# fnzhan/EMLight

Measured on AMD Instinct MI355X. Metric: training images/sec (regression step: DenseNet-BC fwd + Sinkhorn loss + bwd + Adam), higher is better.
Workload: dtype f32; 1 GPU; RegressionNetwork train step, BASELINE configs[1]; per_gpu_batch=64, global_batch=64, anchors=128, parallelism=single

## Files before the change

emlight_amd/RegressionNetwork/dense_engine_bwd.py:

```python
import ctypes
import os

import torch

from .. import _lib
from .._knobs import knob_choice, knob_flag


def _r16(v):
    return (v + 15) // 16 * 16


def _side_stream(dev, prio):
    if prio <= 0:
        return torch.cuda.Stream(device=dev, priority=prio)
    hip = ctypes.CDLL("libamdhip64.so")
    h = ctypes.c_void_p()
    with torch.cuda.device(dev):
        rc = hip.hipStreamCreateWithPriority(ctypes.byref(h), ctypes.c_uint(1), ctypes.c_int(prio))
    if rc != 0:
        raise RuntimeError("hipStreamCreateWithPriority failed (%d)" % rc)
    return torch.cuda.ExternalStream(h.value, device=dev)


def _masked_stream(dev, n_cu, keep):
    hip = ctypes.CDLL("libamdhip64.so")
    words = (n_cu + 31) // 32
    mask = (ctypes.c_uint32 * words)()
    for i in range(n_cu):
        if keep(i):
            mask[i // 32] |= 1 << (i % 32)
    h = ctypes.c_void_p()
    with torch.cuda.device(dev):
        rc = hip.hipExtStreamCreateWithCUMask(ctypes.byref(h), ctypes.c_uint32(words), mask)
    if rc != 0:
        raise RuntimeError("hipExtStreamCreateWithCUMask failed (%d)" % rc)
    return torch.cuda.ExternalStream(h.value, device=dev)


class _BwdBuffers:
    def __init__(self, enc, ws, dev):
        f32 = dict(dtype=torch.float32, device=dev)
        self.G = [torch.zeros(blk["P"], blk["ld"], **f32) for blk in ws.blocks]
        self.GF = torch.zeros(ws.F.shape[0], ws.F.shape[1], **f32)
        maxP = ws.blocks[0]["P"]
        self.DZ = torch.empty(2, maxP, 48, **f32)
        self.ring = max(1, int(os.environ.get("EML_WGRAD_RING", 4))) if enc.overlap_wgrad(dev) else 1
        self.GF12 = [torch.empty(maxP, 12, **f32) for _ in range(self.ring)]
        self.N12 = torch.empty(maxP, 12, **f32)
        self.TOP = torch.empty(2 * maxP * 12, **f32) if knob_flag("EML_DGRAD_TOP", True) else None
        kp, ko, g = enc.kp_max, max(enc.ko_max, 48), enc.grid_max
        self.Wd = [[torch.empty(lay["Kp"] * 48, **f32) for lay in blk["layers"]] for blk in ws.blocks]
        self.WdT = [torch.empty(blk["trans"]["Kp"] * blk["trans"]["Ko"], **f32) for blk in ws.blocks]
        self.permutes = None
        self.coef = torch.zeros(8, max(kp, ko), **f32)
        self.part2 = torch.zeros(2, g * kp * 2, dtype=torch.float64, device=dev)
        self.partW = torch.empty(g * max(kp * 48, 2 * 27 * 256, 4 * 1024), **f32)
        i32 = dict(dtype=torch.int32, device=dev)
        self.cond = [[torch.zeros(lay["Kp"], **i32) for lay in blk["layers"]] for blk in ws.blocks]
        self.condT = [torch.zeros(blk["trans"]["Kp"], **i32) for blk in ws.blocks]
        self.any_ill = torch.zeros(1, **i32)
        self.dg_grid = 128
        self.dg_scratch = torch.empty(self.dg_grid * kp, dtype=torch.float64, device=dev)
        self.side = None
        if enc.overlap_wgrad(dev):
            m = int(os.environ.get("EML_CU_SPLIT", 0))
            self.main_masked = None
            if m > 1:
                n_cu = torch.cuda.get_device_properties(dev).multi_processor_count
                self.side = _masked_stream(dev, n_cu, lambda i: i % m == m - 1)
                self.main_masked = _masked_stream(dev, n_cu, lambda i: i % m != m - 1)
# ... 49 lines not shown
        mod_ = getattr(f, "denseblock%d" % (bi_ + 1))
        for l_, lay_ in enumerate(blk_["layers"]):
            items.append((getattr(mod_, "denselayer%d" % (l_ + 1)).conv1.weight, bw.Wd[bi_][l_], 2, 48, lay_["Cin"],
                          lay_["Kp"], 48))
        tr_ = blk_["trans"]
        items.append((getattr(f, "transition%d" % (bi_ + 1)).conv.weight, bw.WdT[bi_], 2, tr_["Cout"], blk_["Ctot"],
                      tr_["Kp"], tr_["Ko"]))
    bw.permutes.launch(L, st, items)
    params = enc.param_list()
    if need_params is None:
        need_params = [True] * len(params)
    from .._dist import grad_slot
    grads = {}
    for q, need in zip(params, need_params):
        slot = grad_slot(q) if need else None
        grads[id(q)] = slot if slot is not None else torch.empty_like(q)
    gr = lambda q: p(grads[id(q)])
    coefs = [tuple(bw.coef[3 * k + i] for i in range(3)) for k in range(2)]
    cA, cB, cC = coefs[0]
    sB, sC = bw.coef[6], bw.coef[7]

    direct = knob_choice("EML_DGAMMA_DIRECT", "always", ("always", "never")) != "never"
    c3_fold = knob_flag("EML_C3_FOLD", True)
    bw.any_ill.zero_()

    def dgamma_direct(blk, X_ld, Pin, Hin, Win, pool, DY, ld_dy, Zr, ld_z, co, Cout, conv, Cin, scale1, shift1, cond, bn):
        if not direct:
            return
        a, b, c = co if co is not None else (None, None, None)
        _lib.check(L.eml_dense_bn_dgamma_direct_f32(
            p(blk["X"]), X_ld, Pin, Hin, Win, pool, p(DY), ld_dy, p(Zr), ld_z, p(a), p(b), p(c), Cout, p(conv.weight), Cin,
            p(scale1), p(shift1), p(blk["mean"]), p(blk["istd"]), p(cond), p(bw.dg_scratch), gr(bn.weight), bw.dg_grid, st),
            "eml_dense_bn_dgamma_direct_f32")

    def finalize(R, pstride, count, bn, mean, istd, C, Cpad, coef=0, s_acc=None, src=None, c_lo=0, c_hi=None, conv=None,
                 cond=None):
        a, b, c = coefs[coef] if coef is not None else (None, None, None)
        wargs = (p(bn.bias), p(conv.weight), gr(conv.weight), conv.weight.shape[0]) if conv is not None else (None, None, None, 0)
        _lib.check(L.eml_dense_bn_bwd_finalize_f32(
            p(part if src is None else src), R, pstride, float(count), p(bn.weight), p(mean), p(istd), C, Cpad, 1,
            gr(bn.weight), gr(bn.bias), p(a), p(b), p(c),
            p(sB) if s_acc is not None else None, p(sC) if s_acc is not None else None, int(bool(s_acc)),
            c_lo, Cpad if c_hi is None else c_hi, *wargs, p(cond), p(bw.any_ill) if cond is not None else None, st),
            "eml_dense_bn_bwd_finalize_f32")

    def parr(tensors):
# ... 29 lines not shown
        _lib.check(L.eml_dense_conv1x1_bwd_data_f32(
            p(dY), ld_dy, p(tr["T"]), Ko, p(cA), p(cB), p(cC), Ko, p(bw.WdT[bi]), None, ld, p(tr["scale"]),
            p(tr["shift"]), None, None, Pn, Hb, Wb, 1, kpt, p(Gbuf), ld, 0, p(part), G, p(tr["mask16"]), st),
            "eml_dense_conv1x1_bwd_data_f32")
        finalize(G, 2 * kpt, P, T.norm, blk["mean"], blk["istd"], ctot, kpt, coef=None, s_acc=False, conv=T.conv,
                 cond=bw.condT[bi])
        dgamma_direct(blk, ld, P, Hb, Wb, 1, dY, ld_dy, tr["T"], Ko, coefs[0], cout, T.conv, ctot, tr["scale"], tr["shift"],
                      bw.condT[bi], T.norm)
        def conv2_backward(l, slot, n12=False, narrow_lo=None, top=False):
            lay = blk["layers"][l]
            Lm = getattr(mod, "denselayer%d" % (l + 1))
            cin, kp, z, dz = lay["Cin"], lay["Kp"], blk["Z"][l], bw.DZ[slot]
            gsrc = (p(bw.N12), 12, 0) if n12 else (p(top2[1]), 12, 0) if top else (p(Gbuf), ld, cin)
            r = ring[0] = (ring[0] + 1) % bw.ring
            if bw.side is not None and bw.ev_done[r] is not None:
                main.wait_event(bw.ev_done[r])
            fold = (bw.side is None and c3_fold
                    and L.eml_dense_conv3x3_bwd_fused_supported(gsrc[1], gsrc[2], ld, cin) == 1)
            q = ws.drop_plan[bi][l] if ws.drop_plan is not None else 0.0
            drop = (ws.drop_key, gl0 + l, q) if q > 0 else ()
            if fold:
                fn = "eml_dense_conv3x3_bwd_fused_drop_f32" if drop else "eml_dense_conv3x3_bwd_fused_f32"
                _lib.check(getattr(L, fn)(*gsrc, p(Lm.conv2.weight), p(z), p(lay["zmean"]), p(lay["zistd"]), p(dz), B, Hb, Wb,
                                          p(part), G3d, p(blk["X"]), ld, cin, p(sB), p(sC), p(bw.GF12[r]), p(lay["scale2"]),
                                          p(lay["shift2"]), p(bw.partW), gr(Lm.conv2.weight), *drop, st), fn)
            else:
                fn = "eml_dense_conv3x3_bwd_data_drop_f32" if drop else "eml_dense_conv3x3_bwd_data_f32"
                _lib.check(getattr(L, fn)(*gsrc, p(Lm.conv2.weight), p(z), p(lay["zmean"]), p(lay["zistd"]), p(dz), B, Hb, Wb,
                                          p(part), G3d, p(blk["X"]), ld, cin, p(sB), p(sC), p(bw.GF12[r]), *drop, st), fn)
            if fold:
                pass
            elif bw.side is None:
                _lib.check(L.eml_dense_conv3x3_bwd_weight_f32(p(bw.GF12[r]), 12, 0, p(z), p(lay["scale2"]),
                                                              p(lay["shift2"]), B, Hb, Wb, p(bw.partW),
                                                              gr(Lm.conv2.weight), G3, st),
                           "eml_dense_conv3x3_bwd_weight_f32")
            else:
                bw.ev_ready[r].record(main)
                bw.side.wait_event(bw.ev_ready[r])
                _lib.check(L.eml_dense_conv3x3_bwd_weight_f32(p(bw.GF12[r]), 12, 0, p(z), p(lay["scale2"]),
                                                              p(lay["shift2"]), B, Hb, Wb, p(bw.partW3[r]),
                                                              gr(Lm.conv2.weight), G3s, st_side),
                           "eml_dense_conv3x3_bwd_weight_f32")
                if bw.ev_done[r] is None:
                    bw.ev_done[r] = torch.cuda.Event()
                bw.ev_done[r].record(bw.side)
            finalize(G3d, 96, P, Lm.norm2, lay["zmean"], lay["zistd"], 48, 48, coef=slot)
            a, b, c = coefs[slot]
            _lib.check(L.eml_dense_conv1x1_bwd_weight_f32(
                p(blk["X"]), ld, P, Hb, Wb, 0, kp, cin, p(lay["scale1"]), p(lay["shift1"]), p(dz), 48, p(z), 48,
                p(a), p(b), p(c), 48, p(bw.partW), gr(Lm.conv1.weight), Gw, p(dz),
                *((p(Lm.conv1.weight), narrow_lo, *((p(top2[0]), 12) if top else (p(Gbuf), ld)), p(bw.N12),
                   p(bw.part2[slot])) if narrow_lo is not None
                  else (None, 0, None, 0, None, None)), st), "eml_dense_conv1x1_bwd_weight_f32")
            return Lm

        def dgrad(layers, slots, k_lo, k_hi, top=False):
            lays = [blk["layers"][l] for l in layers]
            if top:
                _lib.check(L.eml_dense_conv1x1_bwd_data_multi_top_f32(
                    parr([bw.DZ[s_] for s_ in slots]), parr([bw.Wd[bi][l_] for l_ in layers]),
                    parr([y["scale1"] for y in lays]), parr([y["shift1"] for y in lays]),
                    parr([bw.part2[s_] for s_ in slots]), (ctypes.c_int * len(layers))(*[y["Kp"] for y in lays]),
# ... 80 lines not shown
```

emlight_amd/csrc/dense_bwd.hip:

```cpp
#include "eml_common.h"
#include "eml_dropout.h"

#include <cstdint>
#include <cstdlib>
#include <type_traits>

namespace {

using f32x4 = __attribute__((ext_vector_type(4))) float;

__device__ __forceinline__ f32x4 mfma16(float a, float b, f32x4 c) {
  return __builtin_amdgcn_mfma_f32_16x16x4f32(a, b, c, 0, 0, 0);
}
__device__ __forceinline__ float f4c(const float4& v, int t) { return t == 0 ? v.x : t == 1 ? v.y : t == 2 ? v.z : v.w; }
__device__ __forceinline__ double shfl_xor_d(double v, int m) { return __shfl_xor(v, m, 64); }

constexpr int kTH = 8, kTW = 32, kHH = kTH + 2, kHW = kTW + 2;

constexpr int kPSG = 14;
constexpr int kBD = 512;
constexpr int kGRows = 2;
constexpr int kGPass = kHH / kGRows;

template <bool FUSE, bool WIDE, int TH, bool DROP = false>
// ... 420 lines not shown
#pragma unroll
  for (int i = 0; i < 7; ++i) {
    const int idx = w4 + 4 * i;
    if (idx < 27) {
#pragma unroll
      for (int g = 0; g < 4; ++g)
        partial[((((size_t)blockIdx.x * 2 + half) * 27 + idx) * 16 + 4 * kk + g) * 16 + r] = acc[i][g];
    }
  }
}


#ifdef EML_STAMPS
__device__ unsigned long long eml_c3_stamps[8];
#define EML_C3_STAMP(slot)                                                   \
  do {                                                                       \
    const unsigned long long now_ = __builtin_readcyclecounter();            \
    st_acc[slot] += now_ - st_last;                                          \
    st_last = now_;                                                          \
  } while (0)
#else
#define EML_C3_STAMP(slot) do {} while (0)
#endif
template <bool A16, bool DROP = false>
__global__ __launch_bounds__(512, 2) void conv3x3_bwd_fused_kernel(
    const float* __restrict__ G, int ldg, int c0, const float* __restrict__ W2, const float* __restrict__ Z,
    const float* __restrict__ zmean, const float* __restrict__ zistd, float* __restrict__ DZ, int B, int H, int W,
    double* __restrict__ partials , const float* __restrict__ Xb, int ldx, int cx,
    const float* __restrict__ sB, const float* __restrict__ sC, float* __restrict__ GF,
    const float* __restrict__ scale2, const float* __restrict__ shift2, float* __restrict__ partialW ,
    eml::DropKey dk) {
  extern __shared__ __attribute__((aligned(16))) float smem[];
  constexpr int kGT = kHH * kHW * kPSG;
  float* g_l = smem;
  float* z_l = g_l + 2 * kGT;
  float* w_l = z_l + kHH * kHW * kPSW;
  float* coef_l = w_l + 27 * 3 * 64;
  double* red = reinterpret_cast<double*>(coef_l + 32);
  const int tid = threadIdx.x, lane = tid & 63, wave = tid >> 6;
  const int r = lane & 15, kk = lane >> 4;
  const int half = wave >> 2, w4 = wave & 3;

  for (int e = tid; e < 27 * 3 * 64; e += 512) {
    const int l = e & 63, g3 = e >> 6, n = g3 % 3, ts = g3 / 3, s3 = ts % 3, tap = ts / 3;
    w_l[e] = W2[((size_t)(4 * s3 + (l >> 4)) * 48 + 16 * n + (l & 15)) * 9 + tap];
  }
  if (tid < 24) coef_l[tid] = tid < 12 ? sB[cx + tid] : sC[cx + tid - 12];
// ... 17 lines not shown
  for (int it = 0; it < 2; ++it) {
    const int t = min(tid + 512 * it, kWideItems - 1), hp = t / 3;
    w_q[it] = t - 3 * hp;
    w_hy[it] = hp / kHW;
    w_hx[it] = hp - w_hy[it] * kHW;
  }
  float4 gt4[2], xt4[2];
  const int s_hx = min(tid / 12, kHW - 1), s_q = tid % 12;
  const float4 sc = *reinterpret_cast<const float4*>(scale2 + 4 * s_q);
  const float4 sh = *reinterpret_cast<const float4*>(shift2 + 4 * s_q);
  const int s_dst = s_hx * kPSW + 4 * s_q;
  float4 zt[kHH];
  const float* s_src = Z;
  int s_y0 = 0;
  bool s_col = false;
  auto stage_begin = [&](int tile) {
    const int b = tile / (ty_n * tx_n), rem = tile - b * (ty_n * tx_n);
    const int ty = rem / tx_n, tx = rem - ty * tx_n;
#pragma unroll
    for (int it = 0; it < 2; ++it) {
      const int gy = ty * kTH - 1 + w_hy[it], gx = tx * kTW - 1 + w_hx[it];
      w_ok[it] = gy >= 0 && gy < H && gx >= 0 && gx < W;
      w_pix[it] = (b * H + min(max(gy, 0), H - 1)) * W + min(max(gx, 0), W - 1);
      w_own[it] = w_ok[it] && w_hy[it] >= 1 && w_hy[it] <= kTH && w_hx[it] >= 1 && w_hx[it] <= kTW;
    }
    const int gx = tx * kTW - 1 + s_hx;
    s_y0 = ty * kTH - 1;
    s_col = gx >= 0 && gx < W;
    s_src = Z + ((size_t)b * H * W + min(max(gx, 0), W - 1)) * 48 + 4 * s_q;
  };
  auto g_load = [&](int it) {
    const float* gp = G + (size_t)w_pix[it] * ldg + c0 + 4 * w_q[it];
    const float* xp = Xb + (size_t)w_pix[it] * ldx + cx + 4 * w_q[it];
    if constexpr (A16) {
      gt4[it] = *reinterpret_cast<const float4*>(gp);
      xt4[it] = *reinterpret_cast<const float4*>(xp);
    } else {
      const float2 g0 = *reinterpret_cast<const float2*>(gp), g1 = *reinterpret_cast<const float2*>(gp + 2);
      const float2 x0 = *reinterpret_cast<const float2*>(xp), x1 = *reinterpret_cast<const float2*>(xp + 2);
      gt4[it] = make_float4(g0.x, g0.y, g1.x, g1.y);
      xt4[it] = make_float4(x0.x, x0.y, x1.x, x1.y);
    }
  };
  auto g_commit = [&](int it, float* dst) {
    const float4 fb4 = *reinterpret_cast<const float4*>(coef_l + 4 * w_q[it]);
    const float4 fc4 = *reinterpret_cast<const float4*>(coef_l + 12 + 4 * w_q[it]);
    float4 v;
    v.x = fmaf(fb4.x, xt4[it].x, gt4[it].x) + fc4.x;
    v.y = fmaf(fb4.y, xt4[it].y, gt4[it].y) + fc4.y;
    v.z = fmaf(fb4.z, xt4[it].z, gt4[it].z) + fc4.z;
    v.w = fmaf(fb4.w, xt4[it].w, gt4[it].w) + fc4.w;
    if constexpr (DROP) v = eml::drop4(dk, (unsigned)w_pix[it], (unsigned)w_q[it], v);
    if (!w_ok[it]) v = make_float4(0.f, 0.f, 0.f, 0.f);
    float* d = dst + (w_hy[it] * kHW + w_hx[it]) * kPSG + 4 * w_q[it];
    *reinterpret_cast<float2*>(d) = make_float2(v.x, v.y);
    *reinterpret_cast<float2*>(d + 2) = make_float2(v.z, v.w);
    if (w_own[it]) *reinterpret_cast<float4*>(GF + (size_t)w_pix[it] * 12 + 4 * w_q[it]) = v;
  };
  auto z_load = [&](int it) {
    zt[it] = *reinterpret_cast<const float4*>(s_src + (size_t)min(max(s_y0 + it, 0), H - 1) * W * 48);
  };
  auto z_commit = [&](int it, int y0, bool col) {
    const bool ok = col && y0 + it >= 0 && y0 + it < H;
    float4 v;
    v.x = ok ? fmaf(zt[it].x, sc.x, sh.x) : 0.f;
    v.y = ok ? fmaf(zt[it].y, sc.y, sh.y) : 0.f;
    v.z = ok ? fmaf(zt[it].z, sc.z, sh.z) : 0.f;
    v.w = ok ? fmaf(zt[it].w, sc.w, sh.w) : 0.f;
    *reinterpret_cast<float4*>(z_l + s_dst + it * kHW * kPSW) = v;
  };

  int tile = blockIdx.x, cur = 0;
  __syncthreads();
  if (tile < ntiles) {
    stage_begin(tile);
    g_load(0);
    g_load(1);
#pragma unroll
    for (int it = 0; it < kHH; ++it) z_load(it);
    g_commit(0, g_l);
// ... 131 lines not shown
#pragma unroll
  for (int i = 0; i < 7; ++i) {
    const int idx = w4 + 4 * i;
    if (idx < 27) {
#pragma unroll
      for (int g = 0; g < 4; ++g)
        partialW[((((size_t)blockIdx.x * 2 + half) * 27 + idx) * 16 + 4 * kk + g) * 16 + r] = accw[i][g];
    }
  }
  __syncthreads();
  if (tid < 48) {
    double t1 = 0.0, t2 = 0.0;
#pragma unroll
    for (int w8 = 0; w8 < 8; ++w8) {
      t1 += red[(w8 * 48 + tid) * 2 + 0];
      t2 += red[(w8 * 48 + tid) * 2 + 1];
    }
    partials[(size_t)blockIdx.x * 96 + 2 * tid + 0] = t1;
    partials[(size_t)blockIdx.x * 96 + 2 * tid + 1] = (double)zistd[tid] * (t2 - (double)zmean[tid] * t1);
  }
}


template <bool A16, bool DROP = false>
__global__ __launch_bounds__(512, 2) void conv3x3_bwd_fused_tp_kernel(
    const float* __restrict__ G, int ldg, int c0, const float* __restrict__ W2, const float* __restrict__ Z,
    const float* __restrict__ zmean, const float* __restrict__ zistd, float* __restrict__ DZ, int B, int H, int W,
    double* __restrict__ partials , const float* __restrict__ Xb, int ldx, int cx,
    const float* __restrict__ sB, const float* __restrict__ sC, float* __restrict__ GF,
    const float* __restrict__ scale2, const float* __restrict__ shift2, float* __restrict__ partialW ,
    eml::DropKey dk) {
  extern __shared__ __attribute__((aligned(16))) float smem[];
  constexpr int kGT = kHH * kHW * kPSG;
  constexpr int kZS = 48;
  float* g_l = smem;
  float* z_l = g_l + 2 * kGT;
  float* w_l = z_l + 2 * kTH * kTW * kZS;
  float* coef_l = w_l + 27 * 3 * 64;
  double* red = reinterpret_cast<double*>(coef_l + 32);
  const int tid = threadIdx.x, lane = tid & 63, wave = tid >> 6;
  const int r = lane & 15, kk = lane >> 4;

  for (int e = tid; e < 27 * 3 * 64; e += 512) {
    const int l = e & 63, g3 = e >> 6, n = g3 % 3, ts = g3 / 3, s3 = ts % 3, tap = ts / 3;
    w_l[e] = W2[((size_t)(4 * s3 + (l >> 4)) * 48 + 16 * n + (l & 15)) * 9 + tap];
  }
  if (tid < 24) coef_l[tid] = tid < 12 ? sB[cx + tid] : sC[cx + tid - 12];
// ... 25 lines not shown
#pragma unroll
  for (int it = 0; it < 2; ++it) {
    const int t = min(tid + 512 * it, kWideItems - 1), hp = t / 3;
    w_q[it] = t - 3 * hp;
    w_hy[it] = hp / kHW;
    w_hx[it] = hp - w_hy[it] * kHW;
  }
  f32x4 gt4[2], xt4[2];
  constexpr int kZI = kTH * kTW * 12 / 512;
  int z_pq[kZI];
#pragma unroll
  for (int it = 0; it < kZI; ++it) {
    const int t = tid + 512 * it;
    z_pq[it] = ((t / 12) << 4) | (t % 12);
  }
  auto stage_begin = [&](int tile) {
    const int b = tile / (ty_n * tx_n), rem = tile - b * (ty_n * tx_n);
    const int ty = rem / tx_n, tx = rem - ty * tx_n;
#pragma unroll
    for (int it = 0; it < 2; ++it) {
      const int gy = ty * kTH - 1 + w_hy[it], gx = tx * kTW - 1 + w_hx[it];
      w_ok[it] = gy >= 0 && gy < H && gx >= 0 && gx < W;
      w_pix[it] = (b * H + min(max(gy, 0), H - 1)) * W + min(max(gx, 0), W - 1);
      w_own[it] = w_ok[it] && w_hy[it] >= 1 && w_hy[it] <= kTH && w_hx[it] >= 1 && w_hx[it] <= kTW;
    }
  };
  auto g_load = [&](int it) {
    const float* gp = G + (size_t)w_pix[it] * ldg + c0 + 4 * w_q[it];
    const float* xp = Xb + (size_t)w_pix[it] * ldx + cx + 4 * w_q[it];
    if constexpr (A16) {
      asm volatile("global_load_dwordx4 %0, %1, off" : "=&v"(gt4[it]) : "v"(gp) : "memory");
      asm volatile("global_load_dwordx4 %0, %1, off" : "=&v"(xt4[it]) : "v"(xp) : "memory");
    } else {
      const float2 g0 = *reinterpret_cast<const float2*>(gp), g1 = *reinterpret_cast<const float2*>(gp + 2);
      const float2 x0 = *reinterpret_cast<const float2*>(xp), x1 = *reinterpret_cast<const float2*>(xp + 2);
      gt4[it] = f32x4{g0.x, g0.y, g1.x, g1.y};
      xt4[it] = f32x4{x0.x, x0.y, x1.x, x1.y};
    }
  };
  auto g_wait = [&]() {
    if constexpr (A16)
      asm volatile("s_waitcnt vmcnt(0)" : "+v"(gt4[0]), "+v"(xt4[0]), "+v"(gt4[1]), "+v"(xt4[1]) :: "memory");
  };
  auto g_commit = [&](int it, float* dst) {
    const float4 fb4 = *reinterpret_cast<const float4*>(coef_l + 4 * w_q[it]);
    const float4 fc4 = *reinterpret_cast<const float4*>(coef_l + 12 + 4 * w_q[it]);
    float4 v;
    v.x = fmaf(fb4.x, xt4[it][0], gt4[it][0]) + fc4.x;
    v.y = fmaf(fb4.y, xt4[it][1], gt4[it][1]) + fc4.y;
    v.z = fmaf(fb4.z, xt4[it][2], gt4[it][2]) + fc4.z;
    v.w = fmaf(fb4.w, xt4[it][3], gt4[it][3]) + fc4.w;
    if constexpr (DROP) v = eml::drop4(dk, (unsigned)w_pix[it], (unsigned)w_q[it], v);
    if (!w_ok[it]) v = make_float4(0.f, 0.f, 0.f, 0.f);
    float* d = dst + (w_hy[it] * kHW + w_hx[it]) * kPSG + 4 * w_q[it];
    *reinterpret_cast<float2*>(d) = make_float2(v.x, v.y);
    *reinterpret_cast<float2*>(d + 2) = make_float2(v.z, v.w);
    gt4[it] = f32x4{v.x, v.y, v.z, v.w};
  };
  auto g_store = [&](int it) {
    if (w_own[it]) *reinterpret_cast<float4*>(GF + ((unsigned)w_pix[it] * 12u + 4u * (unsigned)w_q[it])) = make_float4(gt4[it][0], gt4[it][1], gt4[it][2], gt4[it][3]);
  };
  auto z_dma = [&](int it, int b, int y0, int x0, int buf) {
    const int pix = z_pq[it] >> 4, q = z_pq[it] & 15;
    const int gy = min(y0 + (pix >> 5), H - 1), gx = min(x0 + (pix & 31), W - 1);
    const float* src = Z + ((size_t)(b * H + gy) * W + gx) * 48 + 4 * q;
    unsigned keep;
    const unsigned dst = __builtin_amdgcn_readfirstlane(
        (unsigned)(size_t)(const __attribute__((address_space(3))) char*)(z_l + buf * (kTH * kTW * kZS) + 4 * (64 * wave + 512 * it)));
    asm volatile("s_mov_b32 %0, m0\n\ts_mov_b32 m0, %2\n\ts_nop 0\n\tglobal_load_lds_dwordx4 %1, off\n\ts_mov_b32 m0, %0"
                 : "=&s"(keep) : "v"(src), "s"(dst) : "memory");
  };

  int tile = blockIdx.x, cur = 0;
  __syncthreads();
  if (tile < ntiles) {
    stage_begin(tile);
    g_load(0);
    g_load(1);
    {
      const int b = tile / (ty_n * tx_n), rem = tile - b * (ty_n * tx_n);
#pragma unroll
      for (int it = 0; it < kZI; ++it) z_dma(it, b, (rem / tx_n) * kTH, (rem % tx_n) * kTW, 0);
// ... 1901 lines not shown
                     (size_t)27 * 256, 1, 0, 0, 0, dW2);
  return eml::check_launch("eml_dense_conv3x3_bwd_weight_f32(reduce)");
}

#ifdef EML_STAMPS
extern "C" int eml_c3_read_stamps(unsigned long long* out, int reset) {
  if (hipMemcpyFromSymbol(out, HIP_SYMBOL(eml_c3_stamps), 8 * sizeof(unsigned long long)) != hipSuccess) return -1;
  if (reset) {
    const unsigned long long z[8] = {0};
    if (hipMemcpyToSymbol(HIP_SYMBOL(eml_c3_stamps), z, sizeof(z)) != hipSuccess) return -1;
  }
  return 0;
}
#endif
extern "C" int eml_dense_conv3x3_bwd_fused_supported(int ldg, int c0, int ldx, int cx) {
  return ((ldg & 1) == 0 && (c0 & 1) == 0 && (ldx & 1) == 0 && (cx & 1) == 0) ? 1 : 0;
}
template <bool DROP>
static int conv3x3_bwd_fused_launch(const char* name, const float* G, int ldg, int c0, const float* W2, const float* Z,
                                    const float* zmean, const float* zistd, float* DZ, int B, int H, int W, double* partials,
                                    int grid, const float* X, int ldx, int cx, const float* sB, const float* sC, float* GF,
                                    const float* scale2, const float* shift2, float* partialW, float* dW2, eml::DropKey dk,
                                    eml_stream_t stream) {
  if (!G || !W2 || !Z || !zmean || !zistd || !DZ || !partials || !X || !sB || !sC || !GF || !scale2 || !shift2 || !partialW ||
      !dW2 || B < 1 || H < 1 || W < 1 || grid < 1 || cx < 0)
    return eml::fail(EML_EINVAL, "%s: bad arguments", name);
  const auto al16 = [](const void* q) { return (reinterpret_cast<uintptr_t>(q) & 15) == 0; };
  if (!eml_dense_conv3x3_bwd_fused_supported(ldg, c0, ldx, cx) || !al16(G) || !al16(X) || !al16(GF) || !al16(Z) || !al16(scale2) ||
      !al16(shift2))
    return eml::fail(EML_EINVAL, "%s: needs even ldg, c0, ldx, cx and 16-byte aligned buffers", name);
  const bool a16 = (ldg & 3) == 0 && (c0 & 3) == 0 && (ldx & 3) == 0 && (cx & 3) == 0;
#ifndef EML_C3_WTP
#define EML_C3_WTP 1
#endif
#if EML_C3_WTP
  const size_t lds = (size_t)(2 * kHH * kHW * kPSG + 2 * kTH * kTW * 48 + 27 * 3 * 64 + 32) * sizeof(float) + 8 * 48 * 2 * sizeof(double);
  if (a16) {
    EML_ENSURE_LDS((&conv3x3_bwd_fused_tp_kernel<true, DROP>), lds);
    hipLaunchKernelGGL((conv3x3_bwd_fused_tp_kernel<true, DROP>), dim3(grid), dim3(512), lds, (hipStream_t)stream, G, ldg, c0, W2, Z,
                       zmean, zistd, DZ, B, H, W, partials, X, ldx, cx, sB, sC, GF, scale2, shift2, partialW, dk);
  } else {
    EML_ENSURE_LDS((&conv3x3_bwd_fused_tp_kernel<false, DROP>), lds);
    hipLaunchKernelGGL((conv3x3_bwd_fused_tp_kernel<false, DROP>), dim3(grid), dim3(512), lds, (hipStream_t)stream, G, ldg, c0, W2, Z,
                       zmean, zistd, DZ, B, H, W, partials, X, ldx, cx, sB, sC, GF, scale2, shift2, partialW, dk);
  }
  int rc = eml::check_launch(name);
  if (rc) return rc;
  hipLaunchKernelGGL(reduce_rows_kernel, dim3(21 * 256 / 64), dim3(256), 0, (hipStream_t)stream, partialW, grid,
                     (size_t)21 * 256, 3, 0, 0, 0, dW2);
  return eml::check_launch(DROP ? "eml_dense_conv3x3_bwd_fused_drop_f32(reduce)" : "eml_dense_conv3x3_bwd_fused_f32(reduce)");
#else
  const size_t lds = (size_t)(2 * kHH * kHW * kPSG + kHH * kHW * kPSW + 27 * 3 * 64 + 32) * sizeof(float) + 8 * 48 * 2 * sizeof(double);
  if (a16) {
    EML_ENSURE_LDS((&conv3x3_bwd_fused_kernel<true, DROP>), lds);
    hipLaunchKernelGGL((conv3x3_bwd_fused_kernel<true, DROP>), dim3(grid), dim3(512), lds, (hipStream_t)stream, G, ldg, c0, W2, Z, zmean,
                       zistd, DZ, B, H, W, partials, X, ldx, cx, sB, sC, GF, scale2, shift2, partialW, dk);
  } else {
    EML_ENSURE_LDS((&conv3x3_bwd_fused_kernel<false, DROP>), lds);
    hipLaunchKernelGGL((conv3x3_bwd_fused_kernel<false, DROP>), dim3(grid), dim3(512), lds, (hipStream_t)stream, G, ldg, c0, W2, Z, zmean,
                       zistd, DZ, B, H, W, partials, X, ldx, cx, sB, sC, GF, scale2, shift2, partialW, dk);
  }
  int rc = eml::check_launch(name);
  if (rc) return rc;
  hipLaunchKernelGGL(reduce_rows_kernel, dim3(27 * 256 / 64), dim3(256), 0, (hipStream_t)stream, partialW, 2 * grid,
                     (size_t)27 * 256, 1, 0, 0, 0, dW2);
  return eml::check_launch(DROP ? "eml_dense_conv3x3_bwd_fused_drop_f32(reduce)" : "eml_dense_conv3x3_bwd_fused_f32(reduce)");
#endif
}

extern "C" int eml_dense_conv3x3_bwd_fused_f32(const float* G, int ldg, int c0, const float* W2, const float* Z,
                                               const float* zmean, const float* zistd, float* DZ, int B, int H, int W,
                                               double* partials, int grid, const float* X, int ldx, int cx,
                                               const float* sB, const float* sC, float* GF, const float* scale2,
                                               const float* shift2, float* partialW, float* dW2, eml_stream_t stream) {
  return conv3x3_bwd_fused_launch<false>("eml_dense_conv3x3_bwd_fused_f32", G, ldg, c0, W2, Z, zmean, zistd, DZ, B, H, W, partials,
                                         grid, X, ldx, cx, sB, sC, GF, scale2, shift2, partialW, dW2, eml::DropKey{}, stream);
}

extern "C" int eml_dense_conv3x3_bwd_fused_drop_f32(const float* G, int ldg, int c0, const float* W2, const float* Z,
                                                    const float* zmean, const float* zistd, float* DZ, int B, int H, int W,
                                                    double* partials, int grid, const float* X, int ldx, int cx,
                                                    const float* sB, const float* sC, float* GF, const float* scale2,
                                                    const float* shift2, float* partialW, float* dW2, unsigned long long seed,
// ... 397 lines not shown
```

emlight_amd/csrc/dense_fwd.hip:

```cpp
#include "eml_common.h"
#include "eml_dropout.h"

namespace {

using f32x4 = __attribute__((ext_vector_type(4))) float;

__device__ __forceinline__ f32x4 mfma16(float a, float b, f32x4 c) {
  return __builtin_amdgcn_mfma_f32_16x16x4f32(a, b, c, 0, 0, 0);
}
__device__ __forceinline__ float f4c(const float4& v, int t) { return t == 0 ? v.x : t == 1 ? v.y : t == 2 ? v.z : v.w; }

__device__ __forceinline__ float4 bn_relu4(float4 x, float4 s, float4 t) {
  float4 r;
  r.x = fmaxf(fmaf(x.x, s.x, t.x), 0.f);
  r.y = fmaxf(fmaf(x.y, s.y, t.y), 0.f);
  r.z = fmaxf(fmaf(x.z, s.z, t.z), 0.f);
  r.w = fmaxf(fmaf(x.w, s.w, t.w), 0.f);
  return r;
}

__device__ __forceinline__ double shfl_xor_d(double v, int m) { return __shfl_xor(v, m, 64); }

template <int NT>
__device__ __forceinline__ void block_stats_store(double (&s)[NT], double (&q)[NT], double* red ,
// ... 219 lines not shown
        __builtin_amdgcn_fence(__ATOMIC_ACQUIRE, "wavefront");
      }
    }
  }
#ifndef EML_FWD_STATS_LDS
#pragma unroll
  for (int n = 0; n < 3; ++n)
#pragma unroll
    for (int g = 0; g < 4; ++g) {
#pragma unroll
      for (int o = 1; o < 16; o <<= 1) {
        ssum[n][g] += shfl_xor_d(ssum[n][g], o);
        ssq[n][g] += shfl_xor_d(ssq[n][g], o);
      }
      if (r == 0) {
        red[(wave * 48 + 16 * n + 4 * kk + g) * 2 + 0] = ssum[n][g];
        red[(wave * 48 + 16 * n + 4 * kk + g) * 2 + 1] = ssq[n][g];
      }
    }
#endif
  __syncthreads();
  for (int e = tid; e < 96; e += 256)
    partials[(size_t)blockIdx.x * 96 + e] = (red[e] + red[96 + e]) + (red[192 + e] + red[288 + e]);
}

constexpr int kTH = 8, kTW = 32;
constexpr int kHH = kTH + 2, kHW = kTW + 2;
constexpr int kPS = 56;

constexpr int kC3Threads = 512;

template <bool DROP>
__global__ __launch_bounds__(kC3Threads) void conv3x3_fwd_kernel(
    const float* __restrict__ Z, const float* __restrict__ scale2, const float* __restrict__ shift2,
    const float* __restrict__ W2p, float* __restrict__ X, int ldx, int c_out0, int B, int H, int W,
    double* __restrict__ partials, eml::DropKey dk) {
  extern __shared__ __attribute__((aligned(16))) float smem[];
  float* st_l = smem + 2 * kHH * kHW * kPS;
  double* red = reinterpret_cast<double*>(st_l + 96);
  const int tid = threadIdx.x, lane = tid & 63, wave = tid >> 6;
  const int r = lane & 15, kk = lane >> 4;

  if (tid < 48) {
    st_l[tid] = scale2[tid];
    st_l[48 + tid] = shift2[tid];
  }
// ... 665 lines not shown
  hipLaunchKernelGGL(permute_w2_kernel, dim3(27), dim3(256), 0, (hipStream_t)stream, W2, Cout, W2p);
  return eml::check_launch("eml_dense_permute_w2_f32");
}

extern "C" int eml_dense_conv1x1_fwd_f32(const float* X, int ldx, long P, int Hin, int Win, int pool, int Kp,
                                         const float* scale, const float* shift, const float* Wp, int Cout,
                                         float* out, int ldo, double* partials, int grid,
                                         unsigned long long* relu_mask, eml_stream_t stream) {
  if (!X || !scale || !shift || !Wp || !out || !partials || P < 1 || grid < 1 || Kp < 16 || (Kp & 15) || Kp > ldx ||
      (ldx & 3) || Cout < 1)
    return eml::fail(EML_EINVAL, "eml_dense_conv1x1_fwd_f32: bad arguments");
  if (relu_mask && (pool || Cout > 48))
    return eml::fail(EML_EINVAL, "eml_dense_conv1x1_fwd_f32: relu_mask is for dense layers (no pool, Cout <= 48)");
  if (pool && ((Hin & 1) || (Win & 1))) return eml::fail(EML_EINVAL, "eml_dense_conv1x1_fwd_f32: pool needs even H, W");
  static const bool staged_env = [] { const char* v = getenv("EML_FWD_STAGED"); return !(v && v[0] == '0'); }();
  const size_t lds0 = ((size_t)Kp * 48 + 2 * Kp) * sizeof(float) + 4 * 48 * 2 * sizeof(double) +
                      (relu_mask ? (size_t)4 * 16 * (Kp / 16) * sizeof(unsigned long long) : 0);
  const size_t stg_bytes = (size_t)4 * 16 * 52 * sizeof(float);
  const int staged = (staged_env && !pool && Cout == 48 && ldo == 48 && (reinterpret_cast<size_t>(out) & 15) == 0 &&
                      lds0 + stg_bytes <= 80 * 1024) ? 1 : 0;
  const size_t lds = lds0 + (staged ? stg_bytes : 0);
  if (lds > 160 * 1024) return eml::fail(EML_EINVAL, "eml_dense_conv1x1_fwd_f32: Kp=%d does not fit LDS", Kp);
  const int nchunks = (Cout + 47) / 48;
  for (int ch = 0; ch < nchunks; ++ch) {
    const int nv = (Cout - ch * 48 < 48) ? Cout - ch * 48 : 48;
    const float* wp = Wp + (size_t)ch * Kp * 48;
    double* pp = partials + (size_t)ch * grid * 96;
    if (pool) {
      EML_ENSURE_LDS((&conv1x1_fwd_kernel<true, false>), lds);
      hipLaunchKernelGGL((conv1x1_fwd_kernel<true, false>), dim3(grid), dim3(256), lds, (hipStream_t)stream, X, ldx, (int)P, Hin,
                         Win, Kp, scale, shift, wp, out + ch * 48, ldo, nv, pp, nullptr, 0);
    } else if (relu_mask) {
      EML_ENSURE_LDS((&conv1x1_fwd_kernel<false, true>), lds);
      hipLaunchKernelGGL((conv1x1_fwd_kernel<false, true>), dim3(grid), dim3(256), lds, (hipStream_t)stream, X, ldx, (int)P,
                         Hin, Win, Kp, scale, shift, wp, out + ch * 48, ldo, nv, pp, relu_mask, staged);
    } else {
      EML_ENSURE_LDS((&conv1x1_fwd_kernel<false, false>), lds);
      hipLaunchKernelGGL((conv1x1_fwd_kernel<false, false>), dim3(grid), dim3(256), lds, (hipStream_t)stream, X, ldx, (int)P,
                         Hin, Win, Kp, scale, shift, wp, out + ch * 48, ldo, nv, pp, nullptr, staged);
    }
    int rc = eml::check_launch("eml_dense_conv1x1_fwd_f32");
    if (rc) return rc;
  }
  return EML_OK;
}

extern "C" int eml_dense_conv3x3_fwd_f32(const float* Z, const float* scale2, const float* shift2, const float* W2p,
// ... 49 lines not shown
```

Baseline: 555.5 images/s.

## Fuse multi-chunk transition 1x1 conv forward into one pass; skip unused GF12 stores

Adds a wide conv1x1 forward kernel that handles two or three 48-channel output chunks per launch, so a transition conv reads and BN-ReLUs its input once instead of once per chunk. Only the 1x1 convs with more than 48 outputs and no pool or relu mask are affected. The fused conv3x3 backward kernels gain a template flag that skips writing the GF12 gradient buffer when the weight-gradient pass is folded in, and by default that buffer is no longer allocated or passed. The wide kernel holds up to 3x the weight tile in LDS at occupancy 1 and carries larger accumulator arrays, which raises register pressure.

Measured after the change: 561.3 images/s (median of 6 runs). +1.0%, better.

```diff
diff --git a/emlight_amd/RegressionNetwork/dense_engine_bwd.py b/emlight_amd/RegressionNetwork/dense_engine_bwd.py
--- a/emlight_amd/RegressionNetwork/dense_engine_bwd.py
+++ b/emlight_amd/RegressionNetwork/dense_engine_bwd.py
@@ -39,6 +39,11 @@
 
 
 class _BwdBuffers:
+    def gf12(self, r):
+        if self.GF12[r] is None:
+            self.GF12[r] = self._gf12_new()
+        return self.GF12[r]
+
     def __init__(self, enc, ws, dev):
         f32 = dict(dtype=torch.float32, device=dev)
         self.G = [torch.zeros(blk["P"], blk["ld"], **f32) for blk in ws.blocks]
@@ -46,7 +51,8 @@
         maxP = ws.blocks[0]["P"]
         self.DZ = torch.empty(2, maxP, 48, **f32)
         self.ring = max(1, int(os.environ.get("EML_WGRAD_RING", 4))) if enc.overlap_wgrad(dev) else 1
-        self.GF12 = [torch.empty(maxP, 12, **f32) for _ in range(self.ring)]
+        self.GF12 = [None] * self.ring
+        self._gf12_new = lambda: torch.empty(maxP, 12, **f32)
         self.N12 = torch.empty(maxP, 12, **f32)
         self.TOP = torch.empty(2 * maxP * 12, **f32) if knob_flag("EML_DGRAD_TOP", True) else None
         kp, ko, g = enc.kp_max, max(enc.ko_max, 48), enc.grid_max
@@ -142,6 +148,7 @@
 
     direct = knob_choice("EML_DGAMMA_DIRECT", "always", ("always", "never")) != "never"
     c3_fold = knob_flag("EML_C3_FOLD", True)
+    c3_gf = knob_flag("EML_C3_GF", False)
     bw.any_ill.zero_()
 
     def dgamma_direct(blk, X_ld, Pin, Hin, Win, pool, DY, ld_dy, Zr, ld_z, co, Cout, conv, Cin, scale1, shift1, cond, bn):
@@ -217,23 +224,23 @@
             if fold:
                 fn = "eml_dense_conv3x3_bwd_fused_drop_f32" if drop else "eml_dense_conv3x3_bwd_fused_f32"
                 _lib.check(getattr(L, fn)(*gsrc, p(Lm.conv2.weight), p(z), p(lay["zmean"]), p(lay["zistd"]), p(dz), B, Hb, Wb,
-                                          p(part), G3d, p(blk["X"]), ld, cin, p(sB), p(sC), p(bw.GF12[r]), p(lay["scale2"]),
-                                          p(lay["shift2"]), p(bw.partW), gr(Lm.conv2.weight), *drop, st), fn)
+                                          p(part), G3d, p(blk["X"]), ld, cin, p(sB), p(sC), p(bw.gf12(r)) if c3_gf else None,
+                                          p(lay["scale2"]), p(lay["shift2"]), p(bw.partW), gr(Lm.conv2.weight), *drop, st), fn)
             else:
                 fn = "eml_dense_conv3x3_bwd_data_drop_f32" if drop else "eml_dense_conv3x3_bwd_data_f32"
                 _lib.check(getattr(L, fn)(*gsrc, p(Lm.conv2.weight), p(z), p(lay["zmean"]), p(lay["zistd"]), p(dz), B, Hb, Wb,
-                                          p(part), G3d, p(blk["X"]), ld, cin, p(sB), p(sC), p(bw.GF12[r]), *drop, st), fn)
+                                          p(part), G3d, p(blk["X"]), ld, cin, p(sB), p(sC), p(bw.gf12(r)), *drop, st), fn)
             if fold:
                 pass
             elif bw.side is None:
-                _lib.check(L.eml_dense_conv3x3_bwd_weight_f32(p(bw.GF12[r]), 12, 0, p(z), p(lay["scale2"]),
+                _lib.check(L.eml_dense_conv3x3_bwd_weight_f32(p(bw.gf12(r)), 12, 0, p(z), p(lay["scale2"]),
                                                               p(lay["shift2"]), B, Hb, Wb, p(bw.partW),
                                                               gr(Lm.conv2.weight), G3, st),
                            "eml_dense_conv3x3_bwd_weight_f32")
             else:
                 bw.ev_ready[r].record(main)
                 bw.side.wait_event(bw.ev_ready[r])
-                _lib.check(L.eml_dense_conv3x3_bwd_weight_f32(p(bw.GF12[r]), 12, 0, p(z), p(lay["scale2"]),
+                _lib.check(L.eml_dense_conv3x3_bwd_weight_f32(p(bw.gf12(r)), 12, 0, p(z), p(lay["scale2"]),
                                                               p(lay["shift2"]), B, Hb, Wb, p(bw.partW3[r]),
                                                               gr(Lm.conv2.weight), G3s, st_side),
                            "eml_dense_conv3x3_bwd_weight_f32")
diff --git a/emlight_amd/csrc/dense_bwd.hip b/emlight_amd/csrc/dense_bwd.hip
--- a/emlight_amd/csrc/dense_bwd.hip
+++ b/emlight_amd/csrc/dense_bwd.hip
@@ -466,7 +466,7 @@
 #else
 #define EML_C3_STAMP(slot) do {} while (0)
 #endif
-template <bool A16, bool DROP = false>
+template <bool A16, bool DROP = false, bool STORE_GF = true>
 __global__ __launch_bounds__(512, 2) void conv3x3_bwd_fused_kernel(
     const float* __restrict__ G, int ldg, int c0, const float* __restrict__ W2, const float* __restrict__ Z,
     const float* __restrict__ zmean, const float* __restrict__ zistd, float* __restrict__ DZ, int B, int H, int W,
@@ -530,7 +530,7 @@
       const int gy = ty * kTH - 1 + w_hy[it], gx = tx * kTW - 1 + w_hx[it];
       w_ok[it] = gy >= 0 && gy < H && gx >= 0 && gx < W;
       w_pix[it] = (b * H + min(max(gy, 0), H - 1)) * W + min(max(gx, 0), W - 1);
-      w_own[it] = w_ok[it] && w_hy[it] >= 1 && w_hy[it] <= kTH && w_hx[it] >= 1 && w_hx[it] <= kTW;
+      if constexpr (STORE_GF) w_own[it] = w_ok[it] && w_hy[it] >= 1 && w_hy[it] <= kTH && w_hx[it] >= 1 && w_hx[it] <= kTW;
     }
     const int gx = tx * kTW - 1 + s_hx;
     s_y0 = ty * kTH - 1;
@@ -563,7 +563,8 @@
     float* d = dst + (w_hy[it] * kHW + w_hx[it]) * kPSG + 4 * w_q[it];
     *reinterpret_cast<float2*>(d) = make_float2(v.x, v.y);
     *reinterpret_cast<float2*>(d + 2) = make_float2(v.z, v.w);
-    if (w_own[it]) *reinterpret_cast<float4*>(GF + (size_t)w_pix[it] * 12 + 4 * w_q[it]) = v;
+    if constexpr (STORE_GF)
+      if (w_own[it]) *reinterpret_cast<float4*>(GF + (size_t)w_pix[it] * 12 + 4 * w_q[it]) = v;
   };
   auto z_load = [&](int it) {
     zt[it] = *reinterpret_cast<const float4*>(s_src + (size_t)min(max(s_y0 + it, 0), H - 1) * W * 48);
@@ -741,7 +742,7 @@
 }
 
 
-template <bool A16, bool DROP = false>
+template <bool A16, bool DROP = false, bool STORE_GF = true>
 __global__ __launch_bounds__(512, 2) void conv3x3_bwd_fused_tp_kernel(
     const float* __restrict__ G, int ldg, int c0, const float* __restrict__ W2, const float* __restrict__ Z,
     const float* __restrict__ zmean, const float* __restrict__ zistd, float* __restrict__ DZ, int B, int H, int W,
@@ -813,7 +814,7 @@
       const int gy = ty * kTH - 1 + w_hy[it], gx = tx * kTW - 1 + w_hx[it];
       w_ok[it] = gy >= 0 && gy < H && gx >= 0 && gx < W;
       w_pix[it] = (b * H + min(max(gy, 0), H - 1)) * W + min(max(gx, 0), W - 1);
-      w_own[it] = w_ok[it] && w_hy[it] >= 1 && w_hy[it] <= kTH && w_hx[it] >= 1 && w_hx[it] <= kTW;
+      if constexpr (STORE_GF) w_own[it] = w_ok[it] && w_hy[it] >= 1 && w_hy[it] <= kTH && w_hx[it] >= 1 && w_hx[it] <= kTW;
     }
   };
   auto g_load = [&](int it) {
@@ -846,9 +847,10 @@
     float* d = dst + (w_hy[it] * kHW + w_hx[it]) * kPSG + 4 * w_q[it];
     *reinterpret_cast<float2*>(d) = make_float2(v.x, v.y);
     *reinterpret_cast<float2*>(d + 2) = make_float2(v.z, v.w);
-    gt4[it] = f32x4{v.x, v.y, v.z, v.w};
+    if constexpr (STORE_GF) gt4[it] = f32x4{v.x, v.y, v.z, v.w};
   };
   auto g_store = [&](int it) {
+    if constexpr (!STORE_GF) return;
     if (w_own[it]) *reinterpret_cast<float4*>(GF + ((unsigned)w_pix[it] * 12u + 4u * (unsigned)w_q[it])) = make_float4(gt4[it][0], gt4[it][1], gt4[it][2], gt4[it][3]);
   };
   auto z_dma = [&](int it, int b, int y0, int x0, int buf) {
@@ -2796,7 +2798,7 @@
                                     int grid, const float* X, int ldx, int cx, const float* sB, const float* sC, float* GF,
                                     const float* scale2, const float* shift2, float* partialW, float* dW2, eml::DropKey dk,
                                     eml_stream_t stream) {
-  if (!G || !W2 || !Z || !zmean || !zistd || !DZ || !partials || !X || !sB || !sC || !GF || !scale2 || !shift2 || !partialW ||
+  if (!G || !W2 || !Z || !zmean || !zistd || !DZ || !partials || !X || !sB || !sC || !scale2 || !shift2 || !partialW ||
       !dW2 || B < 1 || H < 1 || W < 1 || grid < 1 || cx < 0)
     return eml::fail(EML_EINVAL, "%s: bad arguments", name);
   const auto al16 = [](const void* q) { return (reinterpret_cast<uintptr_t>(q) & 15) == 0; };
@@ -2810,13 +2812,25 @@
 #if EML_C3_WTP
   const size_t lds = (size_t)(2 * kHH * kHW * kPSG + 2 * kTH * kTW * 48 + 27 * 3 * 64 + 32) * sizeof(float) + 8 * 48 * 2 * sizeof(double);
   if (a16) {
-    EML_ENSURE_LDS((&conv3x3_bwd_fused_tp_kernel<true, DROP>), lds);
-    hipLaunchKernelGGL((conv3x3_bwd_fused_tp_kernel<true, DROP>), dim3(grid), dim3(512), lds, (hipStream_t)stream, G, ldg, c0, W2, Z,
-                       zmean, zistd, DZ, B, H, W, partials, X, ldx, cx, sB, sC, GF, scale2, shift2, partialW, dk);
+    if (GF) {
+      EML_ENSURE_LDS((&conv3x3_bwd_fused_tp_kernel<true, DROP, true>), lds);
+      hipLaunchKernelGGL((conv3x3_bwd_fused_tp_kernel<true, DROP, true>), dim3(grid), dim3(512), lds, (hipStream_t)stream, G, ldg, c0, W2, Z,
+                         zmean, zistd, DZ, B, H, W, partials, X, ldx, cx, sB, sC, GF, scale2, shift2, partialW, dk);
+    } else {
+      EML_ENSURE_LDS((&conv3x3_bwd_fused_tp_kernel<true, DROP, false>), lds);
+      hipLaunchKernelGGL((conv3x3_bwd_fused_tp_kernel<true, DROP, false>), dim3(grid), dim3(512), lds, (hipStream_t)stream, G, ldg, c0, W2, Z,
+                         zmean, zistd, DZ, B, H, W, partials, X, ldx, cx, sB, sC, GF, scale2, shift2, partialW, dk);
+    }
   } else {
-    EML_ENSURE_LDS((&conv3x3_bwd_fused_tp_kernel<false, DROP>), lds);
-    hipLaunchKernelGGL((conv3x3_bwd_fused_tp_kernel<false, DROP>), dim3(grid), dim3(512), lds, (hipStream_t)stream, G, ldg, c0, W2, Z,
-                       zmean, zistd, DZ, B, H, W, partials, X, ldx, cx, sB, sC, GF, scale2, shift2, partialW, dk);
+    if (GF) {
+      EML_ENSURE_LDS((&conv3x3_bwd_fused_tp_kernel<false, DROP, true>), lds);
+      hipLaunchKernelGGL((conv3x3_bwd_fused_tp_kernel<false, DROP, true>), dim3(grid), dim3(512), lds, (hipStream_t)stream, G, ldg, c0, W2, Z,
+                         zmean, zistd, DZ, B, H, W, partials, X, ldx, cx, sB, sC, GF, scale2, shift2, partialW, dk);
+    } else {
+      EML_ENSURE_LDS((&conv3x3_bwd_fused_tp_kernel<false, DROP, false>), lds);
+      hipLaunchKernelGGL((conv3x3_bwd_fused_tp_kernel<false, DROP, false>), dim3(grid), dim3(512), lds, (hipStream_t)stream, G, ldg, c0, W2, Z,
+                         zmean, zistd, DZ, B, H, W, partials, X, ldx, cx, sB, sC, GF, scale2, shift2, partialW, dk);
+    }
   }
   int rc = eml::check_launch(name);
   if (rc) return rc;
@@ -2826,13 +2840,25 @@
 #else
   const size_t lds = (size_t)(2 * kHH * kHW * kPSG + kHH * kHW * kPSW + 27 * 3 * 64 + 32) * sizeof(float) + 8 * 48 * 2 * sizeof(double);
   if (a16) {
-    EML_ENSURE_LDS((&conv3x3_bwd_fused_kernel<true, DROP>), lds);
-    hipLaunchKernelGGL((conv3x3_bwd_fused_kernel<true, DROP>), dim3(grid), dim3(512), lds, (hipStream_t)stream, G, ldg, c0, W2, Z, zmean,
-                       zistd, DZ, B, H, W, partials, X, ldx, cx, sB, sC, GF, scale2, shift2, partialW, dk);
+    if (GF) {
+      EML_ENSURE_LDS((&conv3x3_bwd_fused_kernel<true, DROP, true>), lds);
+      hipLaunchKernelGGL((conv3x3_bwd_fused_kernel<true, DROP, true>), dim3(grid), dim3(512), lds, (hipStream_t)stream, G, ldg, c0, W2, Z, zmean,
+                         zistd, DZ, B, H, W, partials, X, ldx, cx, sB, sC, GF, scale2, shift2, partialW, dk);
+    } else {
+      EML_ENSURE_LDS((&conv3x3_bwd_fused_kernel<true, DROP, false>), lds);
+      hipLaunchKernelGGL((conv3x3_bwd_fused_kernel<true, DROP, false>), dim3(grid), dim3(512), lds, (hipStream_t)stream, G, ldg, c0, W2, Z, zmean,
+                         zistd, DZ, B, H, W, partials, X, ldx, cx, sB, sC, GF, scale2, shift2, partialW, dk);
+    }
   } else {
-    EML_ENSURE_LDS((&conv3x3_bwd_fused_kernel<false, DROP>), lds);
-    hipLaunchKernelGGL((conv3x3_bwd_fused_kernel<false, DROP>), dim3(grid), dim3(512), lds, (hipStream_t)stream, G, ldg, c0, W2, Z, zmean,
-                       zistd, DZ, B, H, W, partials, X, ldx, cx, sB, sC, GF, scale2, shift2, partialW, dk);
+    if (GF) {
+      EML_ENSURE_LDS((&conv3x3_bwd_fused_kernel<false, DROP, true>), lds);
+      hipLaunchKernelGGL((conv3x3_bwd_fused_kernel<false, DROP, true>), dim3(grid), dim3(512), lds, (hipStream_t)stream, G, ldg, c0, W2, Z, zmean,
+                         zistd, DZ, B, H, W, partials, X, ldx, cx, sB, sC, GF, scale2, shift2, partialW, dk);
+    } else {
+      EML_ENSURE_LDS((&conv3x3_bwd_fused_kernel<false, DROP, false>), lds);
+      hipLaunchKernelGGL((conv3x3_bwd_fused_kernel<false, DROP, false>), dim3(grid), dim3(512), lds, (hipStream_t)stream, G, ldg, c0, W2, Z, zmean,
+                         zistd, DZ, B, H, W, partials, X, ldx, cx, sB, sC, GF, scale2, shift2, partialW, dk);
+    }
   }
   int rc = eml::check_launch(name);
   if (rc) return rc;
diff --git a/emlight_amd/csrc/dense_fwd.hip b/emlight_amd/csrc/dense_fwd.hip
--- a/emlight_amd/csrc/dense_fwd.hip
+++ b/emlight_amd/csrc/dense_fwd.hip
@@ -1,3 +1,5 @@
+#include <algorithm>
+
 #include "eml_common.h"
 #include "eml_dropout.h"
 
@@ -265,6 +267,148 @@
   __syncthreads();
   for (int e = tid; e < 96; e += 256)
     partials[(size_t)blockIdx.x * 96 + e] = (red[e] + red[96 + e]) + (red[192 + e] + red[288 + e]);
+}
+
+template <int NT>
+__global__ __launch_bounds__(256, 1) void conv1x1_fwd_wide_kernel(
+    const float* __restrict__ X, int ldx, int P, int Kp, const float* __restrict__ scale, const float* __restrict__ shift,
+    const float* __restrict__ Wp , float* __restrict__ out , int ldo,
+    int n_valid , double* __restrict__ partials, size_t chunk_stride ) {
+  constexpr int NCH = (NT + 2) / 3;
+  extern __shared__ __attribute__((aligned(16))) float smem[];
+  float* wl = smem;
+  float* sl = wl + (size_t)NCH * Kp * 48;
+  float* tl = sl + Kp;
+  double* red = reinterpret_cast<double*>(tl + Kp);
+  const int tid = threadIdx.x, lane = tid & 63, wave = tid >> 6;
+  const int r = lane & 15, kk = lane >> 4;
+
+#pragma unroll 8
+  for (int e = tid; e < NCH * Kp * 12; e += 256)
+    reinterpret_cast<float4*>(wl)[e] = reinterpret_cast<const float4*>(Wp)[e];
+  for (int e = tid; e < Kp; e += 256) {
+    sl[e] = scale[e];
+    tl[e] = shift[e];
+  }
+  for (int e = tid; e < NCH * 4 * 48 * 2; e += 256) red[e] = 0.0;
+  __syncthreads();
+
+  double ssum[NT][4], ssq[NT][4];
+#pragma unroll
+  for (int n = 0; n < NT; ++n)
+#pragma unroll
+    for (int g = 0; g < 4; ++g) ssum[n][g] = ssq[n][g] = 0.0;
+  const int nj = Kp >> 4;
+  const int ntiles = (P + 255) >> 8;
+  const bool vec_ok = (ldo & 3) == 0 && (reinterpret_cast<size_t>(out) & 15) == 0;
+  auto row_ptr = [&](int tile, int m) -> const float* {
+    const int pm = min(tile * 256 + wave * 64 + 16 * m + r, P - 1);
+    return X + (size_t)pm * ldx + 4 * kk;
+  };
+  float4 xa[4], xb[4];
+  int tile = blockIdx.x;
+  if (tile < ntiles) {
+#pragma unroll
+    for (int m = 0; m < 4; ++m) {
+      xa[m] = *reinterpret_cast<const float4*>(row_ptr(tile, m));
+      xb[m] = *reinterpret_cast<const float4*>(row_ptr(tile, m) + 16);
+    }
+  }
+  for (; tile < ntiles; tile += gridDim.x) {
+    const int p0 = tile * 256 + wave * 64;
+    const float* rp[4];
+    const float* rpn[4];
+#pragma unroll
+    for (int m = 0; m < 4; ++m) {
+      rp[m] = row_ptr(tile, m);
+      rpn[m] = row_ptr(min(tile + (int)gridDim.x, ntiles - 1), m);
+    }
+    f32x4 acc[4][NT];
+#pragma unroll
+    for (int m = 0; m < 4; ++m)
+#pragma unroll
+      for (int n = 0; n < NT; ++n) acc[m][n] = f32x4{0.f, 0.f, 0.f, 0.f};
+
+#pragma unroll 2
+    for (int j = 0; j < nj; ++j) {
+      const float4 s4 = *reinterpret_cast<const float4*>(sl + 16 * j + 4 * kk);
+      const float4 t4 = *reinterpret_cast<const float4*>(tl + 16 * j + 4 * kk);
+      float4 a[4], xc[4];
+      const bool wrap = j + 2 >= nj;
+#pragma unroll
+      for (int m = 0; m < 4; ++m) {
+        xc[m] = xa[m];
+        xa[m] = xb[m];
+      }
+#pragma unroll
+      for (int m = 0; m < 4; ++m)
+        xb[m] = *reinterpret_cast<const float4*>(wrap ? rpn[m] + 16 * (j + 2 - nj) : rp[m] + 16 * (j + 2));
+      __builtin_amdgcn_sched_barrier(0);
+#pragma unroll
+      for (int m = 0; m < 4; ++m) a[m] = bn_relu4(xc[m], s4, t4);
+      float4 bw[NT];
+#pragma unroll
+      for (int n = 0; n < NT; ++n)
+        bw[n] = *reinterpret_cast<const float4*>(wl + (size_t)(n / 3) * Kp * 48 + ((size_t)(j * 4 + kk) * 48 + 16 * (n % 3) + r) * 4);
+#pragma unroll
+      for (int t = 0; t < 4; ++t)
+#pragma unroll
+        for (int m = 0; m < 4; ++m)
+#pragma unroll
+          for (int n = 0; n < NT; ++n) acc[m][n] = mfma16(f4c(bw[n], t), f4c(a[m], t), acc[m][n]);
+    }
+#pragma unroll
+    for (int n = 0; n < NT; ++n) {
+      const int c4 = 16 * n + 4 * kk;
+      float ls[4] = {0.f, 0.f, 0.f, 0.f}, lq[4] = {0.f, 0.f, 0.f, 0.f};
+#pragma unroll
+      for (int m = 0; m < 4; ++m) {
+        const int p = p0 + 16 * m + r;
+        const bool pv = p < P;
+#pragma unroll
+        for (int g = 0; g < 4; ++g) {
+          const float v = (pv && c4 + g < n_valid) ? acc[m][n][g] : 0.f;
+          ls[g] += v;
+          lq[g] = fmaf(v, v, lq[g]);
+        }
+        if (pv) {
+          float* dst = out + (size_t)p * ldo + c4;
+          if (vec_ok && c4 + 4 <= n_valid) {
+            *reinterpret_cast<float4*>(dst) = make_float4(acc[m][n][0], acc[m][n][1], acc[m][n][2], acc[m][n][3]);
+          } else {
+#pragma unroll
+            for (int g = 0; g < 4; ++g)
+              if (c4 + g < n_valid) dst[g] = acc[m][n][g];
+          }
+        }
+      }
+#pragma unroll
+      for (int g = 0; g < 4; ++g) {
+        ssum[n][g] += (double)ls[g];
+        ssq[n][g] += (double)lq[g];
+      }
+    }
+  }
+#pragma unroll
+  for (int n = 0; n < NT; ++n)
+#pragma unroll
+    for (int g = 0; g < 4; ++g) {
+#pragma unroll
+      for (int o = 1; o < 16; o <<= 1) {
+        ssum[n][g] += shfl_xor_d(ssum[n][g], o);
+        ssq[n][g] += shfl_xor_d(ssq[n][g], o);
+      }
+      if (r == 0) {
+        red[(((n / 3) * 4 + wave) * 48 + 16 * (n % 3) + 4 * kk + g) * 2 + 0] = ssum[n][g];
+        red[(((n / 3) * 4 + wave) * 48 + 16 * (n % 3) + 4 * kk + g) * 2 + 1] = ssq[n][g];
+      }
+    }
+  __syncthreads();
+  for (int e = tid; e < NCH * 96; e += 256) {
+    const int c = e / 96, ee = e - 96 * c;
+    const double* rc = red + c * 384;
+    partials[c * chunk_stride + (size_t)blockIdx.x * 96 + ee] = (rc[ee] + rc[96 + ee]) + (rc[192 + ee] + rc[288 + ee]);
+  }
 }
 
 constexpr int kTH = 8, kTW = 32;
@@ -976,7 +1120,44 @@
   const size_t lds = lds0 + (staged ? stg_bytes : 0);
   if (lds > 160 * 1024) return eml::fail(EML_EINVAL, "eml_dense_conv1x1_fwd_f32: Kp=%d does not fit LDS", Kp);
   const int nchunks = (Cout + 47) / 48;
-  for (int ch = 0; ch < nchunks; ++ch) {
+  static const bool onepass_env = [] { const char* v = getenv("EML_TRANS_ONEPASS"); return !(v && v[0] == '0'); }();
+  int per = 1;
+  if (onepass_env && !pool && !relu_mask && nchunks > 1 && Kp >= 32) {
+    const size_t per_chunk = (size_t)Kp * 48 * sizeof(float) + 4 * 48 * 2 * sizeof(double), fixed = (size_t)2 * Kp * sizeof(float);
+    const int nfit = (int)std::min<size_t>(3, (160 * 1024 - fixed) / per_chunk);
+    if (nfit >= 2) {
+      const int ndisp = (nchunks + nfit - 1) / nfit;
+      per = (nchunks + ndisp - 1) / ndisp;
+    }
+  }
+  int ch = 0;
+  while (per > 1 && nchunks - ch >= 2) {
+    const int take = std::min(per, nchunks - ch);
+    const int nv = std::min(Cout - ch * 48, 48 * take), nt = (nv + 15) / 16;
+    const size_t wlds = (size_t)take * ((size_t)Kp * 48 * sizeof(float) + 4 * 48 * 2 * sizeof(double)) + (size_t)2 * Kp * sizeof(float);
+    const float* wp = Wp + (size_t)ch * Kp * 48;
+    double* pp = partials + (size_t)ch * grid * 96;
+#define EML_FWD_WIDE(NT_)                                                                                                     \
+  case NT_:                                                                                                                   \
+    EML_ENSURE_LDS((&conv1x1_fwd_wide_kernel<NT_>), wlds);                                                                    \
+    hipLaunchKernelGGL((conv1x1_fwd_wide_kernel<NT_>), dim3(grid), dim3(256), wlds, (hipStream_t)stream, X, ldx, (int)P, Kp,  \
+                       scale, shift, wp, out + ch * 48, ldo, nv, pp, (size_t)grid * 96);                                      \
+    break
+    switch (nt) {
+      EML_FWD_WIDE(4);
+      EML_FWD_WIDE(5);
+      EML_FWD_WIDE(6);
+      EML_FWD_WIDE(7);
+      EML_FWD_WIDE(8);
+      EML_FWD_WIDE(9);
+      default: return eml::fail(EML_EINVAL, "eml_dense_conv1x1_fwd_f32: internal: %d output tiles in %d chunks", nt, take);
+    }
+#undef EML_FWD_WIDE
+    int rc = eml::check_launch("eml_dense_conv1x1_fwd_f32(wide)");
+    if (rc) return rc;
+    ch += take;
+  }
+  for (; ch < nchunks; ++ch) {
     const int nv = (Cout - ch * 48 < 48) ? Cout - ch * 48 : 48;
     const float* wp = Wp + (size_t)ch * Kp * 48;
     double* pp = partials + (size_t)ch * grid * 96;
```
